# rmazzier/OpenSetGaitRecognition_PCAA

Measured on AMD Instinct MI355X. Metric: gait sequences/sec (train step), higher is better.
Workload: dtype bf16; 1 GPU; PCAA V4 train step (enc+dec+disc fwd/bwd, WGAN-GP, Chamfer, 2x Adam), B=64/GPU T=30 N=128 C=4 K=8, BASELINE config[1]; global_batch=64, precision=bf16, parallelism=dp1, sync_bn=False, finite_loss=True, hip_graph=False, decoder_update=fused wgrad+adam

## Files before the change

include/pcaa_hip.h:

```cpp
#ifndef PCAA_HIP_H
#define PCAA_HIP_H

#include <stddef.h>

#ifdef __cplusplus
extern "C" {
#endif

#define PCAA_ABI_VERSION 27

#define PCAA_OK 0
#define PCAA_ERR_INVALID_ARG 1
#define PCAA_ERR_LAUNCH 2

#define PCAA_F32 0
#define PCAA_BF16 1
#define PCAA_SPLIT_F16 2

#define PCAA_LAYOUT_KC 0
#define PCAA_LAYOUT_RC 1

#define PCAA_ACT_NONE 0
#define PCAA_ACT_ELU 1

const char* pcaa_last_error(void);
int pcaa_abi_version(void);

#define PCAA_GEMM_KERNEL_F32_TILE128 0
#define PCAA_GEMM_KERNEL_BF16_SMALL 1
#define PCAA_GEMM_KERNEL_BF16_STAGED 2
#define PCAA_GEMM_KERNEL_V2_KC 3
#define PCAA_GEMM_KERNEL_V2_RC 4
int pcaa_gemm(int math,
              const void* A, int a_dtype, int a_layout, long lda,
              const void* B, int b_dtype, int b_layout, long ldb,
              void* C, int c_dtype, long ldc,
              int M, int N, int K,
              const float* bias, double* colstats, int nrep,
              int split_k, int accumulate, void* stream);

int pcaa_gemm_num_splits(int math, int K, int split_k);
int pcaa_gemm_route(int math,
                    const void* A, int a_dtype, int a_layout, long lda,
                    const void* B, int b_dtype, int b_layout, long ldb,
                    const void* C, int c_dtype, long ldc,
                    int M, int N, int K,
                    const float* bias, const double* colstats, int nrep,
                    int split_k, int accumulate, long slab_stride);
int pcaa_gemm_split3_route(const void* A, const void* B, int layout, long lda, long ldb, const void* C, long ldc, int M,
                           int N, int K, const double* colstats, int nrep, int split_k, long c_split_stride, float out_scale);
int pcaa_gemm_last_kernel(void);
int pcaa_gemm_group_rc_f32(int n, const void* const* A, const void* const* B, void* const* C, const int* M,
                           const int* N, const int* K, const int* split_k, void* stream);
int pcaa_gemm_group_rc_f32_slabs(int n, const void* const* A, const void* const* B, void* const* slabs, const int* M,
                                 const int* N, const int* K, const int* split_k, void* stream);
int pcaa_gemm_v2_enable(int on);
int pcaa_gemm_slabs(int math,
                    const void* A, int a_dtype, int a_layout, long lda,
                    const void* B, int b_dtype, int b_layout, long ldb,
                    float* slabs, long slab_stride, int M, int N, int K, int split_k, void* stream);
int pcaa_gemm_affine_elu(const void* A, long lda, const void* W, long ldw, void* out, long ldo,
                         const float* scale, const float* shift, int M, int N, int K, int pool_rows,
                         void* stream);
int pcaa_gemm_dgrad_bn_supported(int M, int N, int K);
int pcaa_gemm_dgrad_bn(const void* dy, long lddy, const void* Wt, long ldw, const void* y, void* dz, long ld,
                       const float* scale, const float* shift, const float* mean, const float* rstd,
                       double* stats, int nrep, int M, int N, int K,
                       const float* x, int xc, const float* W1, void* stream);
int pcaa_bn_bwd_dy_split(const float* dz, const float* y, void* dy_img, const float* coef, long rows, int ch,
                         float img_scale, void* stream);
int pcaa_gemm_dgrad_bn_split3(const void* dy_img, long lddy, const void* Wt_img, long ldw, const float* y, float* dz,
                              long ld, const float* scale, const float* shift, const float* mean, const float* rstd,
                              double* stats, int nrep, int M, int N, int K, float out_scale, void* stream);
int pcaa_timing_events_create(void** start, void** stop);
int pcaa_timing_events_destroy(void* start, void* stop);
int pcaa_time_next_gemm(void* start, void* stop);
int pcaa_timing_pending(void);
int pcaa_timing_elapsed_ms(void* start, void* stop, float* ms);
int pcaa_splitk_reduce(const float* slabs, int nsplit, long slab_stride, long n, float* out,
                       int accumulate, void* stream);
int pcaa_splitk_reduce_stats(const float* slabs, int nsplit, long slab_stride, float* out,
                             double* stats, int nrep, long rows, int ch, void* stream);

int pcaa_pointnet_in_fwd(const float* x, int C, const float* W, const float* bias, void* y, int y_dtype,
                         long P, int cout, double* stats, int nrep, void* stream);
int pcaa_pointnet_in_wgrad(const void* dy, int dy_dtype, const float* x, int C, float* dW, long P,
                           int cout, void* stream);
int pcaa_pointnet_in_apply(const float* x, int C, const float* W, const float* scale, const float* shift,
                           void* a, int a_dtype, long P, int cout, void* stream);
int pcaa_pointnet_in_bwd_stats(const void* da, int dtype, const float* x, int C, const float* W,
                               const float* scale, const float* shift, const float* mean, const float* rstd,
                               double* stats, int nrep, long P, int cout, void* stream);
int pcaa_pointnet_in_bwd_onepass(const void* da, int dtype, const float* x, int C, const float* W,
                                 const float* scale, const float* shift, const float* mean, const float* rstd,
                                 double* stats, int nrep, float* G, long P, int cout, const double* pivot_mom,
                                 double pivot_inv_count, void* stream);
int pcaa_pointnet_in_bwd_onepass_rows(const void* da, int dtype, const float* x, int C, const float* W,
                                      const float* scale, const float* shift, const float* mean, const float* rstd,
                                      double* stats, int nrep, float* G, long P, int cout, const double* pivot_mom,
                                      double pivot_inv_count, void* stream);
int pcaa_pointnet_in_bwd_g_rows(long P);
int pcaa_points_moments_size(void);
int pcaa_points_moments(const float* x, int C, long P, double* mom, void* stream);
int pcaa_pointnet_in_bwd_combine(const float* G, int nrep, const float* W, const double* mom, const float* coef,
                                 float* dW, int cout, int C, long P, const double* pivot_mom, double pivot_inv_count,
                                 void* stream);
int pcaa_pointnet_in_moment_stats(const double* mom, const float* W, int C, int cout, void* stream);
int pcaa_pointnet_in_bwd_wgrad(const void* da, int dtype, const float* x, int C, const float* W,
                               const float* scale, const float* shift, const float* coef, float* dW,
                               long P, int cout, int dz_is_pre ,
                               void* stream);

int pcaa_cast_bf16(const float* src, void* dst, void* dst_t, int R, int C, void* stream);

int pcaa_bn_finalize(const double* stats, int nrep, long count, const float* lin_bias,
                     const float* gamma, const float* beta,
                     float* running_mean, float* running_var, long long* num_batches_tracked,
                     float momentum, float eps,
                     float* scale, float* shift, float* mean, float* rstd, int ch, void* stream);
int pcaa_bn_eval_coeffs(const float* gamma, const float* beta, const float* running_mean,
                        const float* running_var, const float* lin_bias, float eps, float* scale,
                        float* shift, int ch, void* stream);
int pcaa_bn_act_fwd(const void* y, void* a, int dtype, const float* scale, const float* shift,
                    long rows, int ch, void* stream);
int pcaa_bn_act_meanpool_fwd(const void* y, int dtype, const float* scale, const float* shift,
                             const float* mean, const float* rstd, float* pooled, float* e1, float* e2,
                             long groups, int group_rows, int ch, void* stream);
int pcaa_bn_pool_bwd_stats(const float* dpool, const float* e1, const float* e2, float pool_scale,
                           double* stats, int nrep, long groups, int ch, void* stream);
int pcaa_bn_act_bwd_dz(const void* da, const float* dpool, int group_rows, float pool_scale,
                       const void* y, void* dz, int dtype,
                       const float* scale, const float* shift, const float* mean, const float* rstd,
                       double* stats, int nrep, long rows, int ch, void* stream);
int pcaa_bn_bwd_finalize(const double* stats, int nrep, long count, const float* gamma,
                         const float* mean, const float* rstd,
                         float* coef, float* dgamma, float* dbeta, int ch, void* stream);
int pcaa_bn_bwd_dy(const void* dz, const void* y, void* dy, int dtype, const float* coef,
                   long rows, int ch, void* stream);
int pcaa_bn_eval_moments(const float* running_mean, const float* running_var, const float* lin_bias,
                         float eps, float* mean, float* rstd, int ch, void* stream);
int pcaa_bn_eval_act_bwd(const void* da, const float* dpool, int group_rows, float pool_scale,
                         const void* y, void* dy, int dtype,
                         const float* scale, const float* shift, const float* mean, const float* rstd,
                         double* stats, int nrep, long rows, int ch, void* stream);
int pcaa_bn_eval_bwd_finalize(const double* stats, int nrep, const float* scale,
                              float* dgamma, float* dbeta, float* dbias, int ch, void* stream);
int pcaa_bn_tail_arm_fwd(const double* stats, int nrep, long count, const float* lin_bias,
                         const float* gamma, const float* beta,
                         float* running_mean, float* running_var, long long* num_batches_tracked,
                         float momentum, float eps,
                         float* scale, float* shift, float* mean, float* rstd, int ch, unsigned* counter);
int pcaa_bn_tail_arm_bwd(const double* stats, int nrep, long count, const float* gamma,
                         const float* mean, const float* rstd,
                         float* coef, float* dgamma, float* dbeta, int ch, unsigned* counter);
int pcaa_bn_tail_pending(void);
int pcaa_bn_tail_disarm(void);
int pcaa_bn_bwd_dy_fused(const void* da, const float* dpool, int group_rows, float pool_scale,
                         const void* y, void* dy, int dtype, const float* scale, const float* shift,
                         const float* coef, long rows, int ch, void* stream);

int pcaa_bias_act(float* y, const float* bias, int act, long rows, int cols, void* stream);
int pcaa_elu_bwd_from_out(const float* da, const float* a, float* dz, long n, void* stream);
int pcaa_colsum(const float* x, float* out, long rows, int cols, void* stream);
int pcaa_sum(const float* x, long n, float scale, float* out, void* stream);
int pcaa_rowsum(const float* x, float* out, long rows, int cols, float scale, void* stream);
int pcaa_scale_by_device_scalar(const float* x, const float* s, float* out, long n, void* stream);
int pcaa_scale_rows(const float* x, const float* s, float* out, long rows, int cols, void* stream);
int pcaa_prior_sample(const float* z0, const float* means, const long long* gt, int B, int K, int D,
                      float* z, float* onehot, void* stream);
int pcaa_pack_points(const float* src, long sb, long sc, long st, long sn,
                     float* dst, int B, int C, int T, int N, void* stream);

int pcaa_gather_rows(const void* src, long n_src_rows, long row_bytes, const long long* idx, void* dst,
                     long n_rows, int* err_flag, void* stream);

int pcaa_dtc_im2col(const float* a, float* col, int B, int T, int Cin, int dilation, void* stream);
int pcaa_dtc_col2im(const float* dcol, float* da, int B, int T, int Cin, int dilation, void* stream);

int pcaa_chamfer_fwd_bwd(const float* preds, long p_sb, long p_sc, long p_st, long p_sn,
                         const float* gts, long g_sb, long g_sc, long g_st, long g_sn,
                         int B, int T, int N, int C, float* frame_loss,
                         float* dpreds, long d_sb, long d_sc, long d_st, long d_sn,
                         float grad_scale, const float* grad_per_b, void* stream);
int pcaa_cross_entropy(const float* logits, const long long* target, int B, int K,
                       float* loss, float* dlogits, float grad_scale, long long* preds,
                       int* err_flag, void* stream);

int pcaa_disc_forward(const float* x, const float* label, int B, int K,
                      const float* W1, const float* b1, const float* W2, const float* b2,
                      const float* W3, const float* b3, float* out, void* stream);
int pcaa_disc_backward(const float* x, const float* label, int B, int K,
                       const float* W1, const float* b1, const float* W2, const float* b2,
                       const float* W3, const float* b3, const float* gout,
                       float* dx, float* dlabel,
                       float* dW1, float* db1, float* dW2, float* db2, float* dW3, float* db3,
                       float* workspace, size_t workspace_bytes, void* stream);
int pcaa_disc_backward_backward(const float* x, const float* label, int B, int K,
                                const float* W1, const float* b1, const float* W2, const float* b2,
                                const float* W3, const float* b3, const float* gout, const float* gbar,
                                float* dx2, float* dlabel2, float* dgout,
                                float* dW1, float* db1, float* dW2, float* db2, float* dW3, float* db3,
                                float* workspace, size_t workspace_bytes, void* stream);
size_t pcaa_disc_workspace_bytes(int B, int K);
int pcaa_disc_wgan_gp(const float* z, const float* fv, const float* label, const float* alphas,
                      int B, int K,
                      const float* W1, const float* b1, const float* W2, const float* b2,
                      const float* W3, const float* b3, float gp_weight, float* losses,
                      float* dW1, float* db1, float* dW2, float* db2, float* dW3, float* db3,
                      float* dz, float* workspace, size_t workspace_bytes, void* stream);

int pcaa_joint_likelihood(const float* x, const float* means, int B, int K, int D, double* lik,
                          void* stream);
int pcaa_kvote(const double* lik, const long long* preds, double threshold, int k, int n_labels,
               int n_classes, int n_windows, long long* out, void* stream);

int pcaa_skinny_supported(int M, int N, int K);
int pcaa_skinny_splits(int kind, int M, int N, int K);
int pcaa_skinny_linear_fwd(const float* x, long ldx, const float* W, long ldw, const float* bias, int act,
                           float* y, float* ws, long ws_floats, int M, int N, int K, int nsplit,
                           void* stream);
int pcaa_skinny_linear_dgrad(const float* dz, long lddz, const float* W, long ldw, float* dx,
// ... 173 lines not shown
```

opensetgaitrecognition_pcaa_amd/csrc/elementwise.hip:

```cpp
#include <stdarg.h>

#include "common.h"
#include "bn_tail.h"

static thread_local char g_err[512] = "";
void pcaa_set_error(const char* fmt, ...) {
  va_list ap;
  va_start(ap, fmt);
  vsnprintf(g_err, sizeof(g_err), fmt, ap);
  va_end(ap);
}
extern "C" const char* pcaa_last_error(void) { return g_err; }
static thread_local int* g_range_flag = nullptr;
int* pcaa_range_flag_ptr() { return g_range_flag; }
extern "C" int pcaa_set_range_flag(int* dev_flag) { g_range_flag = dev_flag; return PCAA_OK; }
extern "C" int pcaa_abi_version(void) { return PCAA_ABI_VERSION; }

namespace {

constexpr int ROWS_PER_BLOCK = 128;

inline bool ch_ok(int ch) {
  if (ch < 4 || ch > 1024 || (ch & 3)) return false;
  const int q = ch >> 2;
  return (256 % q) == 0;
}

__device__ __forceinline__ void replica_sums(const double* __restrict__ stats, int nrep, int ch, int c, double& s1,
                                             double& s2) {
  int r = 0;
  for (; r + 8 <= nrep; r += 8) {
    double a[8], b[8];
#pragma unroll
    for (int u = 0; u < 8; ++u) {
      a[u] = stats[((long)(r + u) * 2 + 0) * ch + c];
      b[u] = stats[((long)(r + u) * 2 + 1) * ch + c];
    }
#pragma unroll
    for (int u = 0; u < 8; ++u) { s1 += a[u]; s2 += b[u]; }
  }
  for (; r < nrep; ++r) {
    s1 += stats[((long)r * 2 + 0) * ch + c];
    s2 += stats[((long)r * 2 + 1) * ch + c];
  }
}

__global__ void bn_finalize_kernel(const double* __restrict__ stats, int nrep, double inv_count,
                                   double unbias, const float* __restrict__ lin_bias,
                                   const float* __restrict__ gamma, const float* __restrict__ beta,
                                   float* running_mean, float* running_var, long long* nbt,
                                   float momentum, float eps, float* scale, float* shift,
                                   float* mean_out, float* rstd_out, int ch) {
  const int c = blockIdx.x * blockDim.x + threadIdx.x;
  if (c == 0 && nbt) *nbt += 1;
  if (c >= ch) return;
  double s1 = 0.0, s2 = 0.0;
  replica_sums(stats, nrep, ch, c, s1, s2);
  const double m0 = s1 * inv_count;
  double var = s2 * inv_count - m0 * m0;
  if (var < 0.0) var = 0.0;
  const double mean = m0 + (lin_bias ? (double)lin_bias[c] : 0.0);
  const double rstd = 1.0 / sqrt(var + (double)eps);
  const float sc = (float)((double)gamma[c] * rstd);
  scale[c] = sc;
  shift[c] = (float)((double)beta[c] - m0 * (double)gamma[c] * rstd);
  mean_out[c] = (float)m0;
  rstd_out[c] = (float)rstd;
  if (running_mean) {
    running_mean[c] = (1.f - momentum) * running_mean[c] + momentum * (float)mean;
    running_var[c] = (1.f - momentum) * running_var[c] + momentum * (float)(var * unbias);
  }
}

__global__ void bn_eval_coeffs_kernel(const float* gamma, const float* beta, const float* rm,
                                      const float* rv, const float* lin_bias, float eps, float* scale,
                                      float* shift, int ch) {
  const int c = blockIdx.x * blockDim.x + threadIdx.x;
  if (c >= ch) return;
  const float rstd = 1.f / sqrtf(rv[c] + eps);
  const float sc = gamma[c] * rstd;
  scale[c] = sc;
  shift[c] = beta[c] + ((lin_bias ? lin_bias[c] : 0.f) - rm[c]) * sc;
}

template <typename T>
__global__ __launch_bounds__(256) void bn_act_fwd_kernel(const T* __restrict__ y, T* __restrict__ a,
// ... 511 lines not shown
    long r = i / Cin;
    const int t = (int)(r % T);
    const long b = r / T;
    float acc = 0.f;
#pragma unroll
    for (int tap = 0; tap < 3; ++tap) {
      const int tt = t + (2 - tap) * d;
      if (tt < T) acc += dcol[((b * T + tt) * Cin + ci) * 3 + tap];
    }
    da[i] = acc;
  }
}

template <int U, typename TG = float>
__global__ __launch_bounds__(256) void adam_kernel(float* __restrict__ p, const TG* __restrict__ g,
                                                   float* __restrict__ m, float* __restrict__ v, long n,
                                                   float b1, float b2, float eps, float step_size,
                                                   float inv_bc2_sqrt, float grad_scale,
                                                   const float* __restrict__ coef) {
  if (coef) {
    step_size = coef[0];
    inv_bc2_sqrt = coef[1];
  }
  const long nq = n >> 2;
  const long stride = (long)gridDim.x * 256;
  for (long q0 = (long)blockIdx.x * 256 + threadIdx.x; q0 < nq; q0 += stride * U) {
    f32x4 pv[U], gv[U], mv[U], vv[U];
#pragma unroll
    for (int u = 0; u < U; ++u) {
      const long q = q0 + u * stride;
      if (q < nq) { pv[u] = load4(p + q * 4); gv[u] = load4(g + q * 4); mv[u] = load4(m + q * 4); vv[u] = load4(v + q * 4); }
    }
#pragma unroll
    for (int u = 0; u < U; ++u) {
      const long q = q0 + u * stride;
      if (q >= nq) break;
#pragma unroll
      for (int e = 0; e < 4; ++e) {
        float pe = pv[u][e], me = mv[u][e], ve = vv[u][e];
        adam_update(pe, me, ve, gv[u][e] * grad_scale, b1, b2, eps, step_size, inv_bc2_sqrt);
        pv[u][e] = pe; mv[u][e] = me; vv[u][e] = ve;
      }
      store4(p + q * 4, pv[u]);
      store4(m + q * 4, mv[u]);
      store4(v + q * 4, vv[u]);
    }
  }
  if (blockIdx.x == 0 && threadIdx.x < (n & 3)) {
    const long i = (nq << 2) + threadIdx.x;
    float pp = p[i], mm = m[i], vv = v[i];
    adam_update(pp, mm, vv, (float)g[i] * grad_scale, b1, b2, eps, step_size, inv_bc2_sqrt);
    m[i] = mm;
    v[i] = vv;
    p[i] = pp;
  }
}

__global__ void adam_coef_kernel(int* __restrict__ step, float* __restrict__ coef, float lr, float b1, float b2) {
  const int t = *step + 1;
  *step = t;
  const double bc1 = 1.0 - pow((double)b1, (double)t);
  const double bc2 = 1.0 - pow((double)b2, (double)t);
  coef[0] = (float)((double)lr / bc1);
  coef[1] = (float)(1.0 / sqrt(bc2));
}

inline int grid_for(long work_items, int per_block = 256, int cap = 256 * 8) {
  long g = cdiv(work_items, per_block);
  if (g < 1) g = 1;
  if (g > cap) g = cap;
  return (int)g;
}

inline int col_invariant_grid(long nquads, int qpr) {
  int a = qpr, b = 256;
  while (b) { const int t = a % b; a = b; b = t; }
  const int unit = qpr / a;
  long g = cdiv(nquads, 256);
  if (g > 2048) g = 2048;
  g = cdiv(g, unit) * unit;
  return (int)g;
}

}

extern "C" int pcaa_bn_finalize(const double* stats, int nrep, long count, const float* lin_bias,
                                const float* gamma, const float* beta, float* running_mean,
                                float* running_var, long long* num_batches_tracked, float momentum,
                                float eps, float* scale, float* shift, float* mean, float* rstd,
                                int ch, void* stream) {
  PCAA_CHECK_ARG(stats && gamma && beta && scale && shift && mean && rstd, "pcaa_bn_finalize: null pointer");
  PCAA_CHECK_ARG(nrep >= 1 && count >= 1 && ch >= 1, "pcaa_bn_finalize: bad sizes");
  PCAA_CHECK_ARG((running_mean == nullptr) == (running_var == nullptr), "pcaa_bn_finalize: running stats must come together");
  const double unbias = count > 1 ? (double)count / (double)(count - 1) : 1.0;
  hipLaunchKernelGGL(bn_finalize_kernel, dim3((unsigned)cdiv(ch, 256)), dim3(256), 0, as_stream(stream),
                     stats, nrep, 1.0 / (double)count, unbias, lin_bias, gamma, beta, running_mean,
                     running_var, num_batches_tracked, momentum, eps, scale, shift, mean, rstd, ch);
  PCAA_RETURN_LAUNCH_STATUS("pcaa_bn_finalize");
}

extern "C" int pcaa_bn_eval_coeffs(const float* gamma, const float* beta, const float* running_mean,
                                   const float* running_var, const float* lin_bias, float eps, float* scale,
                                   float* shift, int ch, void* stream) {
  PCAA_CHECK_ARG(gamma && beta && running_mean && running_var && scale && shift && ch >= 1, "pcaa_bn_eval_coeffs: bad args");
  hipLaunchKernelGGL(bn_eval_coeffs_kernel, dim3((unsigned)cdiv(ch, 256)), dim3(256), 0, as_stream(stream),
                     gamma, beta, running_mean, running_var, lin_bias, eps, scale, shift, ch);
  PCAA_RETURN_LAUNCH_STATUS("pcaa_bn_eval_coeffs");
}

extern "C" int pcaa_bn_act_fwd(const void* y, void* a, int dtype, const float* scale, const float* shift,
                               long rows, int ch, void* stream) {
  PCAA_CHECK_ARG(y && a && scale && shift, "pcaa_bn_act_fwd: null pointer");
  PCAA_CHECK_ARG(rows >= 1 && ch >= 4 && (ch & 3) == 0, "pcaa_bn_act_fwd: ch must be a multiple of 4");
  const long nq = rows * (ch >> 2);
  PCAA_CHECK_ARG(nq < (1L << 31), "pcaa_bn_act_fwd: tensor too large for 32-bit quad indices");
  const int grid = col_invariant_grid(nq, ch >> 2);
  if (dtype == PCAA_F32)
    hipLaunchKernelGGL(bn_act_fwd_kernel<float>, dim3(grid), dim3(256), 0, as_stream(stream),
                       (const float*)y, (float*)a, scale, shift, (unsigned)nq, (unsigned)(ch >> 2));
  else if (dtype == PCAA_BF16)
    hipLaunchKernelGGL(bn_act_fwd_kernel<bf16_t>, dim3(grid), dim3(256), 0, as_stream(stream),
                       (const bf16_t*)y, (bf16_t*)a, scale, shift, (unsigned)nq, (unsigned)(ch >> 2));
  else { pcaa_set_error("pcaa_bn_act_fwd: bad dtype"); return PCAA_ERR_INVALID_ARG; }
  PCAA_RETURN_LAUNCH_STATUS("pcaa_bn_act_fwd");
}

extern "C" int pcaa_bn_act_fwd_split(const float* y, void* a_img, const float* scale, const float* shift, long rows,
                                     int ch, float img_scale, void* stream) {
  PCAA_CHECK_ARG(y && a_img && scale && shift, "pcaa_bn_act_fwd_split: null pointer");
  PCAA_CHECK_ARG(rows >= 1 && ch >= 4 && (ch & 3) == 0, "pcaa_bn_act_fwd_split: ch must be a multiple of 4");
  const long nq = rows * (ch >> 2);
  PCAA_CHECK_ARG(nq < (1L << 31), "pcaa_bn_act_fwd_split: tensor too large for 32-bit quad indices");
  const int grid = col_invariant_grid(nq, ch >> 2);
  hipLaunchKernelGGL(bn_act_fwd_split_kernel, dim3(grid), dim3(256), 0, as_stream(stream), y, (split_t*)a_img, scale, shift,
                     (unsigned)nq, (unsigned)(ch >> 2), img_scale, pcaa_range_flag_ptr());
  PCAA_RETURN_LAUNCH_STATUS("pcaa_bn_act_fwd_split");
}

extern "C" int pcaa_split_f16(const float* src, void* dst_img, long rows, int ch, int transpose, float img_scale,
                               void* stream) {
  PCAA_CHECK_ARG(src && dst_img && rows >= 1 && ch >= 1, "pcaa_split_f16: bad args");
  long g = cdiv(rows * ch, 256);
  if (g > 4096) g = 4096;
  hipLaunchKernelGGL(split_f16_kernel, dim3((unsigned)g), dim3(256), 0, as_stream(stream), src, (split_t*)dst_img, rows, ch,
                     transpose, img_scale, pcaa_range_flag_ptr());
  PCAA_RETURN_LAUNCH_STATUS("pcaa_split_f16");
}

extern "C" int pcaa_bn_act_meanpool_fwd(const void* y, int dtype, const float* scale, const float* shift,
                                        const float* mean, const float* rstd, float* pooled, float* e1, float* e2,
                                        long groups, int group_rows, int ch, void* stream) {
  PCAA_CHECK_ARG(y && scale && shift && pooled, "pcaa_bn_act_meanpool_fwd: null pointer");
  PCAA_CHECK_ARG(groups >= 1 && group_rows >= 1 && ch_ok(ch), "pcaa_bn_act_meanpool_fwd: ch/4 must divide 256 (ch=%d)", ch);
  const bool train = e1 != nullptr;
  PCAA_CHECK_ARG((e2 != nullptr) == train && (!train || (mean && rstd)),
                 "pcaa_bn_act_meanpool_fwd: e1, e2, mean, rstd come together");
  hipStream_t s = as_stream(stream);
#define LAUNCH_MP(T, TRAIN)                                                                                   \
  hipLaunchKernelGGL((bn_act_meanpool_kernel<T, TRAIN>), dim3((unsigned)groups), dim3(256), 0, s, (const T*)y, \
                     scale, shift, mean, rstd, pooled, e1, e2, group_rows, ch)
  if (dtype == PCAA_BF16 && ch == 1024 && group_rows % 4 == 0 && groups >= 512) {
    const unsigned grid = (unsigned)std::min<long>(groups, 1024);
    if (train)
      hipLaunchKernelGGL(bn_act_meanpool_stream_kernel<true>, dim3(grid), dim3(256), 0, s, (const bf16_t*)y, scale, shift,
                         mean, rstd, pooled, e1, e2, groups, group_rows, ch);
    else
      hipLaunchKernelGGL(bn_act_meanpool_stream_kernel<false>, dim3(grid), dim3(256), 0, s, (const bf16_t*)y, scale, shift,
                         mean, rstd, pooled, e1, e2, groups, group_rows, ch);
  }
  else if (dtype == PCAA_F32) { if (train) LAUNCH_MP(float, true); else LAUNCH_MP(float, false); }
  else if (dtype == PCAA_BF16) { if (train) LAUNCH_MP(bf16_t, true); else LAUNCH_MP(bf16_t, false); }
  else { pcaa_set_error("pcaa_bn_act_meanpool_fwd: bad dtype"); return PCAA_ERR_INVALID_ARG; }
#undef LAUNCH_MP
  PCAA_RETURN_LAUNCH_STATUS("pcaa_bn_act_meanpool_fwd");
}

extern "C" int pcaa_bn_pool_bwd_stats(const float* dpool, const float* e1, const float* e2, float pool_scale,
                                      double* stats, int nrep, long groups, int ch, void* stream) {
  PCAA_CHECK_ARG(dpool && e1 && e2 && stats, "pcaa_bn_pool_bwd_stats: null pointer");
  PCAA_CHECK_ARG(groups >= 1 && ch >= 4 && (ch & 3) == 0 && nrep >= 1, "pcaa_bn_pool_bwd_stats: ch must be a multiple of 4");
  const int gpb = (int)std::max<long>(1, std::min<long>(32, groups / 256));
  hipLaunchKernelGGL(bn_pool_bwd_stats_kernel, dim3((unsigned)cdiv(groups, gpb)), dim3(256), 0, as_stream(stream),
                     dpool, e1, e2, pool_scale, stats, nrep, groups, ch, gpb, pcaa_take_bn_tail(stats));
  PCAA_RETURN_LAUNCH_STATUS("pcaa_bn_pool_bwd_stats");
}

extern "C" int pcaa_bn_act_bwd_dz(const void* da, const float* dpool, int group_rows, float pool_scale,
                                  const void* y, void* dz, int dtype, const float* scale,
                                  const float* shift, const float* mean, const float* rstd,
                                  double* stats, int nrep, long rows, int ch, void* stream) {
  PCAA_CHECK_ARG((da != nullptr) != (dpool != nullptr), "pcaa_bn_act_bwd_dz: exactly one of da / dpool");
  PCAA_CHECK_ARG(y && scale && shift && mean && rstd && stats, "pcaa_bn_act_bwd_dz: null pointer");
  PCAA_CHECK_ARG(rows >= 1 && rows < (1L << 31) && nrep >= 1 && ch_ok(ch),
                 "pcaa_bn_act_bwd_dz: ch/4 must divide 256 (ch=%d), rows < 2^31", ch);
  PCAA_CHECK_ARG(!dpool || group_rows >= 1, "pcaa_bn_act_bwd_dz: bad group_rows");
  const unsigned grid = (unsigned)cdiv(rows, ROWS_PER_BLOCK);
  hipStream_t s = as_stream(stream);
#define LAUNCH_DZ(T, POOL)                                                                       \
// ... 138 lines not shown
  PCAA_CHECK_ARG(rows >= 1 && rows < (1L << 31) && nrep >= 1 && ch_ok(ch),
                 "pcaa_bn_eval_act_bwd: ch/4 must divide 256 (ch=%d), rows < 2^31", ch);
  PCAA_CHECK_ARG(!dpool || group_rows >= 1, "pcaa_bn_eval_act_bwd: bad group_rows");
  PCAA_CHECK_ARG(dy != y, "pcaa_bn_eval_act_bwd: dy may alias da, not y");
  const unsigned grid = (unsigned)cdiv(rows, ROWS_PER_BLOCK);
  hipStream_t s = as_stream(stream);
#define LAUNCH_EV(T, POOL)                                                                         \
  hipLaunchKernelGGL((bn_eval_act_bwd_kernel<T, POOL>), dim3(grid), dim3(256), 0, s, (const T*)da, \
                     dpool, (unsigned)group_rows, pool_scale, (const T*)y, (T*)dy, scale, shift,   \
                     mean, rstd, stats, nrep, rows, ch)
  if (dtype == PCAA_F32) { if (dpool) LAUNCH_EV(float, true); else LAUNCH_EV(float, false); }
  else if (dtype == PCAA_BF16) { if (dpool) LAUNCH_EV(bf16_t, true); else LAUNCH_EV(bf16_t, false); }
  else { pcaa_set_error("pcaa_bn_eval_act_bwd: bad dtype"); return PCAA_ERR_INVALID_ARG; }
#undef LAUNCH_EV
  PCAA_RETURN_LAUNCH_STATUS("pcaa_bn_eval_act_bwd");
}

extern "C" int pcaa_bn_eval_bwd_finalize(const double* stats, int nrep, const float* scale, float* dgamma,
                                         float* dbeta, float* dbias, int ch, void* stream) {
  PCAA_CHECK_ARG(stats && (scale || !dbias), "pcaa_bn_eval_bwd_finalize: null pointer");
  PCAA_CHECK_ARG(nrep >= 1 && ch >= 1, "pcaa_bn_eval_bwd_finalize: bad sizes");
  hipLaunchKernelGGL(bn_eval_bwd_finalize_kernel, dim3((unsigned)cdiv(ch, 256)), dim3(256), 0, as_stream(stream),
                     stats, nrep, scale, dgamma, dbeta, dbias, ch);
  PCAA_RETURN_LAUNCH_STATUS("pcaa_bn_eval_bwd_finalize");
}

namespace {
thread_local BnTail g_tail = {};
}
BnTail pcaa_take_bn_tail(const double* stats) {
  BnTail t = {};
  if (g_tail.kind != 0 && g_tail.stats == stats) {
    t = g_tail;
    g_tail.kind = 0;
  }
  return t;
}
extern "C" int pcaa_bn_tail_arm_fwd(const double* stats, int nrep, long count, const float* lin_bias,
                                    const float* gamma, const float* beta, float* running_mean, float* running_var,
                                    long long* num_batches_tracked, float momentum, float eps, float* scale,
                                    float* shift, float* mean, float* rstd, int ch, unsigned* counter) {
  PCAA_CHECK_ARG(stats && gamma && beta && scale && shift && mean && rstd && counter, "pcaa_bn_tail_arm_fwd: null pointer");
  PCAA_CHECK_ARG(nrep >= 1 && count >= 1 && ch >= 1, "pcaa_bn_tail_arm_fwd: bad sizes");
  PCAA_CHECK_ARG((running_mean == nullptr) == (running_var == nullptr), "pcaa_bn_tail_arm_fwd: running stats must come together");
  BnTail t = {};
  t.kind = 1; t.nrep = nrep; t.ch = ch; t.counter = counter; t.stats = stats;
  t.inv_count = 1.0 / (double)count;
  t.unbias = count > 1 ? (double)count / (double)(count - 1) : 1.0;
  t.lin_bias = lin_bias; t.gamma = gamma; t.beta = beta;
  t.running_mean = running_mean; t.running_var = running_var; t.nbt = num_batches_tracked;
  t.momentum = momentum; t.eps = eps;
  t.scale = scale; t.shift = shift; t.mean = mean; t.rstd = rstd;
  g_tail = t;
  return PCAA_OK;
}
extern "C" int pcaa_bn_tail_arm_bwd(const double* stats, int nrep, long count, const float* gamma, const float* mean,
                                    const float* rstd, float* coef, float* dgamma, float* dbeta, int ch,
                                    unsigned* counter) {
  PCAA_CHECK_ARG(stats && gamma && mean && rstd && coef && counter, "pcaa_bn_tail_arm_bwd: null pointer");
  PCAA_CHECK_ARG(nrep >= 1 && count >= 1 && ch >= 1, "pcaa_bn_tail_arm_bwd: bad sizes");
  BnTail t = {};
  t.kind = 2; t.nrep = nrep; t.ch = ch; t.counter = counter; t.stats = stats;
  t.inv_count = 1.0 / (double)count;
  t.gamma = gamma; t.mean = const_cast<float*>(mean); t.rstd = const_cast<float*>(rstd);
  t.coef = coef; t.dgamma = dgamma; t.dbeta = dbeta;
  g_tail = t;
  return PCAA_OK;
}
void pcaa_rearm_bn_tail(const BnTail& t) {
  if (t.kind != 0) g_tail = t;
}
extern "C" int pcaa_bn_tail_pending(void) { return g_tail.kind != 0 ? 1 : 0; }
extern "C" int pcaa_bn_tail_disarm(void) {
  g_tail.kind = 0;
  return PCAA_OK;
}

extern "C" int pcaa_bn_bwd_dy(const void* dz, const void* y, void* dy, int dtype, const float* coef,
                              long rows, int ch, void* stream) {
  PCAA_CHECK_ARG(dz && y && dy && coef, "pcaa_bn_bwd_dy: null pointer");
  PCAA_CHECK_ARG(rows >= 1 && ch >= 4 && (ch & 3) == 0, "pcaa_bn_bwd_dy: ch must be a multiple of 4");
  const long nq = rows * (ch >> 2);
  PCAA_CHECK_ARG(nq < (1L << 31), "pcaa_bn_bwd_dy: tensor too large for 32-bit quad indices");
  const int grid = col_invariant_grid(nq, ch >> 2);
  if (dtype == PCAA_F32)
    hipLaunchKernelGGL(bn_bwd_dy_kernel<float>, dim3(grid), dim3(256), 0, as_stream(stream), (const float*)dz,
                       (const float*)y, (float*)dy, coef, (unsigned)nq, (unsigned)(ch >> 2), (unsigned)ch);
  else if (dtype == PCAA_BF16)
    hipLaunchKernelGGL(bn_bwd_dy_kernel<bf16_t>, dim3(grid), dim3(256), 0, as_stream(stream), (const bf16_t*)dz,
                       (const bf16_t*)y, (bf16_t*)dy, coef, (unsigned)nq, (unsigned)(ch >> 2), (unsigned)ch);
  else { pcaa_set_error("pcaa_bn_bwd_dy: bad dtype"); return PCAA_ERR_INVALID_ARG; }
  PCAA_RETURN_LAUNCH_STATUS("pcaa_bn_bwd_dy");
}

extern "C" int pcaa_bn_bwd_dy_split(const float* dz, const float* y, void* dy_img, const float* coef, long rows, int ch,
                                    float img_scale, void* stream) {
  PCAA_CHECK_ARG(dz && y && dy_img && coef, "pcaa_bn_bwd_dy_split: null pointer");
  PCAA_CHECK_ARG(rows >= 1 && ch >= 4 && (ch & 3) == 0, "pcaa_bn_bwd_dy_split: ch must be a multiple of 4");
  PCAA_CHECK_ARG((const void*)dz != dy_img && (const void*)y != dy_img, "pcaa_bn_bwd_dy_split: the image cannot alias an input");
  const long nq = rows * (ch >> 2);
  PCAA_CHECK_ARG(nq < (1L << 31), "pcaa_bn_bwd_dy_split: tensor too large for 32-bit quad indices");
  const int grid = col_invariant_grid(nq, ch >> 2);
  hipLaunchKernelGGL(bn_bwd_dy_split_kernel, dim3(grid), dim3(256), 0, as_stream(stream), dz, y, (split_t*)dy_img, coef,
                     (unsigned)nq, (unsigned)(ch >> 2), (unsigned)ch, img_scale, pcaa_range_flag_ptr());
  PCAA_RETURN_LAUNCH_STATUS("pcaa_bn_bwd_dy_split");
}

extern "C" int pcaa_bias_act(float* y, const float* bias, int act, long rows, int cols, void* stream) {
  PCAA_CHECK_ARG(y && rows >= 1 && cols >= 1, "pcaa_bias_act: bad args");
  PCAA_CHECK_ARG(act == PCAA_ACT_NONE || act == PCAA_ACT_ELU, "pcaa_bias_act: bad activation");
  const long n = rows * cols;
  hipLaunchKernelGGL(bias_act_kernel, dim3(grid_for(n)), dim3(256), 0, as_stream(stream), y, bias, act, n, cols);
  PCAA_RETURN_LAUNCH_STATUS("pcaa_bias_act");
}

extern "C" int pcaa_elu_bwd_from_out(const float* da, const float* a, float* dz, long n, void* stream) {
  PCAA_CHECK_ARG(da && a && dz && n >= 1, "pcaa_elu_bwd_from_out: bad args");
  hipLaunchKernelGGL(elu_bwd_from_out_kernel, dim3(grid_for(n)), dim3(256), 0, as_stream(stream), da, a, dz, n);
  PCAA_RETURN_LAUNCH_STATUS("pcaa_elu_bwd_from_out");
}

extern "C" int pcaa_colsum(const float* x, float* out, long rows, int cols, void* stream) {
  PCAA_CHECK_ARG(x && out && rows >= 1 && cols >= 1, "pcaa_colsum: bad args");
  hipLaunchKernelGGL(colsum_kernel, dim3((unsigned)cdiv(cols, 64)), dim3(256), 0, as_stream(stream), x, out, rows, cols);
  PCAA_RETURN_LAUNCH_STATUS("pcaa_colsum");
}

extern "C" int pcaa_sum(const float* x, long n, float scale, float* out, void* stream) {
  PCAA_CHECK_ARG(x && out && n >= 1, "pcaa_sum: bad args");
  hipLaunchKernelGGL(sum_kernel, dim3(1), dim3(1024), 0, as_stream(stream), x, n, scale, out);
  PCAA_RETURN_LAUNCH_STATUS("pcaa_sum");
}

extern "C" int pcaa_rowsum(const float* x, float* out, long rows, int cols, float scale, void* stream) {
  PCAA_CHECK_ARG(x && out && rows >= 1 && cols >= 1, "pcaa_rowsum: bad args");
  hipLaunchKernelGGL(rowsum_kernel, dim3((unsigned)rows), dim3(64), 0, as_stream(stream), x, out, cols, scale);
  PCAA_RETURN_LAUNCH_STATUS("pcaa_rowsum");
}

extern "C" int pcaa_scale_by_device_scalar(const float* x, const float* s, float* out, long n, void* stream) {
  PCAA_CHECK_ARG(x && s && out && n >= 1, "pcaa_scale_by_device_scalar: bad args");
  hipLaunchKernelGGL(scale_dev_kernel, dim3(grid_for(n)), dim3(256), 0, as_stream(stream), x, s, out, n);
  PCAA_RETURN_LAUNCH_STATUS("pcaa_scale_by_device_scalar");
}

extern "C" int pcaa_scale_rows(const float* x, const float* s, float* out, long rows, int cols, void* stream) {
  PCAA_CHECK_ARG(x && s && out && rows >= 1 && cols >= 1, "pcaa_scale_rows: bad args");
  const long n = rows * cols;
  hipLaunchKernelGGL(scale_rows_kernel, dim3(grid_for(n)), dim3(256), 0, as_stream(stream), x, s, out, n, cols);
  PCAA_RETURN_LAUNCH_STATUS("pcaa_scale_rows");
}

extern "C" int pcaa_prior_sample(const float* z0, const float* means, const long long* gt, int B, int K, int D,
                                 float* z, float* onehot, void* stream) {
  PCAA_CHECK_ARG(z0 && means && gt && z && onehot && B >= 1 && K >= 1 && D >= 1, "pcaa_prior_sample: bad args");
  const int n = B * (D > K ? D : K);
  hipLaunchKernelGGL(prior_sample_kernel, dim3((unsigned)cdiv(n, 256)), dim3(256), 0, as_stream(stream), z0, means, gt, B, K, D, z, onehot);
  PCAA_RETURN_LAUNCH_STATUS("pcaa_prior_sample");
}

extern "C" int pcaa_pack_points(const float* src, long sb, long sc, long st, long sn, float* dst,
                                int B, int C, int T, int N, void* stream) {
  PCAA_CHECK_ARG(src && dst && B >= 1 && C >= 1 && T >= 1 && N >= 1, "pcaa_pack_points: bad args");
  const long n = (long)B * C * T * N;
  hipLaunchKernelGGL(pack_points_kernel, dim3(grid_for(n)), dim3(256), 0, as_stream(stream), src, sb, sc, st, sn, dst, B, C, T, N);
  PCAA_RETURN_LAUNCH_STATUS("pcaa_pack_points");
// ... 177 lines not shown
```

Before: 12310 sequences/s.

## Add persistent ring-buffered streaming kernel for bf16 BN act-fwd and bwd-dy

Adds a persistent-grid streaming kernel that keeps per-column coefficients in registers and software-pipelines 16-byte bf16 loads through a small register ring (depth 2-4). The bf16 BN backward dy path and the wide-channel (ch>=1024) activation forward path use it, with nontemporal loads and stores on the backward path. The grid is sized per CU count. The aim is higher memory bandwidth utilisation on these bandwidth-bound elementwise passes, at the cost of extra code paths gated by alignment and channel-divisibility checks and an environment toggle.

After: 12440 sequences/s (median of 6 runs). 1.01x the previous value.

```diff
diff --git a/include/pcaa_hip.h b/include/pcaa_hip.h
--- a/include/pcaa_hip.h
+++ b/include/pcaa_hip.h
@@ -7,7 +7,7 @@
 extern "C" {
 #endif
 
-#define PCAA_ABI_VERSION 27
+#define PCAA_ABI_VERSION 28
 
 #define PCAA_OK 0
 #define PCAA_ERR_INVALID_ARG 1
@@ -137,6 +137,16 @@
                          float* coef, float* dgamma, float* dbeta, int ch, void* stream);
 int pcaa_bn_bwd_dy(const void* dz, const void* y, void* dy, int dtype, const float* coef,
                    long rows, int ch, void* stream);
+#define PCAA_EW_ACT_FWD 0
+#define PCAA_EW_BWD_DY 1
+#define PCAA_EW_BWD_DY_FUSED 2
+#define PCAA_EW_MEANPOOL 3
+#define PCAA_EW_IN_BWD 4
+#define PCAA_EW_IN_APPLY 5
+const char* pcaa_ew_route(int pass, int dtype, long rows, int ch, int aligned);
+int pcaa_ew_wgs_per_cu(int pass);
+int pcaa_ew_ring_depth(int pass);
+int pcaa_ew_stream_set(int on);
 int pcaa_bn_eval_moments(const float* running_mean, const float* running_var, const float* lin_bias,
                          float eps, float* mean, float* rstd, int ch, void* stream);
 int pcaa_bn_eval_act_bwd(const void* da, const float* dpool, int group_rows, float pool_scale,
diff --git a/opensetgaitrecognition_pcaa_amd/csrc/elementwise.hip b/opensetgaitrecognition_pcaa_amd/csrc/elementwise.hip
--- a/opensetgaitrecognition_pcaa_amd/csrc/elementwise.hip
+++ b/opensetgaitrecognition_pcaa_amd/csrc/elementwise.hip
@@ -1,7 +1,10 @@
 #include <stdarg.h>
+
+#include <stdlib.h>
 
 #include "common.h"
 #include "bn_tail.h"
+#include "ew_stream.h"
 
 static thread_local char g_err[512] = "";
 void pcaa_set_error(const char* fmt, ...) {
@@ -679,6 +682,49 @@
   return (int)g;
 }
 
+int g_ew_stream = -1;
+inline bool ew_stream_on() {
+  if (g_ew_stream < 0) {
+    const char* e = getenv("PCAA_EW_STREAM");
+    g_ew_stream = (e && e[0] == '0' && e[1] == 0) ? 0 : 1;
+  }
+  return g_ew_stream != 0;
+}
+inline bool ew_route_stream(int pass, int dtype, long rows, int ch, bool aligned16) {
+  if (!ew_stream_on() || dtype != PCAA_BF16 || rows < 1 || !aligned16 || !ew::ch_ok(ch)) return false;
+  if (pass == PCAA_EW_ACT_FWD) return ch >= 1024;
+  return pass == PCAA_EW_BWD_DY;
+}
+inline bool aligned16(const void* a, const void* b, const void* c) {
+  return (((uintptr_t)a | (uintptr_t)b | (uintptr_t)c) & 15) == 0;
+}
+
+}
+
+int ew::cu_count() {
+  static int n = 0;
+  if (n <= 0) {
+    int dev = 0;
+    if (hipGetDevice(&dev) != hipSuccess || hipDeviceGetAttribute(&n, hipDeviceAttributeMultiprocessorCount, dev) != hipSuccess ||
+        n <= 0)
+      n = 256;
+  }
+  return n;
+}
+
+extern "C" const char* pcaa_ew_route(int pass, int dtype, long rows, int ch, int aligned) {
+  return ew_route_stream(pass, dtype, rows, ch, aligned != 0) ? "stream" : "classic";
+}
+extern "C" int pcaa_ew_wgs_per_cu(int pass) {
+  return pass == PCAA_EW_ACT_FWD ? ew::ActFwdPolicy::K : pass == PCAA_EW_BWD_DY ? ew::BwdDyPolicy::K : 0;
+}
+extern "C" int pcaa_ew_ring_depth(int pass) {
+  return pass == PCAA_EW_ACT_FWD ? ew::ActFwdPolicy::R : pass == PCAA_EW_BWD_DY ? ew::BwdDyPolicy::R : 0;
+}
+extern "C" int pcaa_ew_stream_set(int on) {
+  const int was = ew_stream_on() ? 1 : 0;
+  g_ew_stream = on ? 1 : 0;
+  return was;
 }
 
 extern "C" int pcaa_bn_finalize(const double* stats, int nrep, long count, const float* lin_bias,
@@ -711,6 +757,11 @@
   PCAA_CHECK_ARG(rows >= 1 && ch >= 4 && (ch & 3) == 0, "pcaa_bn_act_fwd: ch must be a multiple of 4");
   const long nq = rows * (ch >> 2);
   PCAA_CHECK_ARG(nq < (1L << 31), "pcaa_bn_act_fwd: tensor too large for 32-bit quad indices");
+  if (ew_route_stream(PCAA_EW_ACT_FWD, dtype, rows, ch, aligned16(y, a, nullptr))) {
+    ew::launch<1, ew::ActFwdPolicy>((const bf16_t*)y, nullptr, (bf16_t*)a, ew::ActFwd{scale, shift}, rows, ch,
+                                    as_stream(stream));
+    PCAA_RETURN_LAUNCH_STATUS("pcaa_bn_act_fwd");
+  }
   const int grid = col_invariant_grid(nq, ch >> 2);
   if (dtype == PCAA_F32)
     hipLaunchKernelGGL(bn_act_fwd_kernel<float>, dim3(grid), dim3(256), 0, as_stream(stream),
@@ -1015,6 +1066,11 @@
   PCAA_CHECK_ARG(rows >= 1 && ch >= 4 && (ch & 3) == 0, "pcaa_bn_bwd_dy: ch must be a multiple of 4");
   const long nq = rows * (ch >> 2);
   PCAA_CHECK_ARG(nq < (1L << 31), "pcaa_bn_bwd_dy: tensor too large for 32-bit quad indices");
+  if (ew_route_stream(PCAA_EW_BWD_DY, dtype, rows, ch, aligned16(dz, y, dy))) {
+    ew::launch<2, ew::BwdDyPolicy>((const bf16_t*)y, (const bf16_t*)dz, (bf16_t*)dy, ew::BwdDy{coef}, rows, ch,
+                                   as_stream(stream));
+    PCAA_RETURN_LAUNCH_STATUS("pcaa_bn_bwd_dy");
+  }
   const int grid = col_invariant_grid(nq, ch >> 2);
   if (dtype == PCAA_F32)
     hipLaunchKernelGGL(bn_bwd_dy_kernel<float>, dim3(grid), dim3(256), 0, as_stream(stream), (const float*)dz,
diff --git a/opensetgaitrecognition_pcaa_amd/csrc/ew_stream.h b/opensetgaitrecognition_pcaa_amd/csrc/ew_stream.h
--- /dev/null
+++ b/opensetgaitrecognition_pcaa_amd/csrc/ew_stream.h
@@ -0,0 +1,117 @@
+#pragma once
+#include "common.h"
+
+namespace ew {
+
+typedef unsigned int u32x2 __attribute__((ext_vector_type(2)));
+typedef unsigned int u32x4 __attribute__((ext_vector_type(4)));
+
+constexpr int OCT = 8;
+
+inline bool ch_ok(int ch) { return ch >= OCT && (ch % OCT) == 0 && ch / OCT <= 256 && (256 % (ch / OCT)) == 0; }
+inline int rows_per_trip(int ch) { return 256 / (ch / OCT); }
+
+__device__ __forceinline__ f32x4 unpack(unsigned lo, unsigned hi) {
+  return f32x4{__uint_as_float(lo << 16), __uint_as_float(lo & 0xffff0000u), __uint_as_float(hi << 16),
+               __uint_as_float(hi & 0xffff0000u)};
+}
+__device__ __forceinline__ u32x2 pack(f32x4 v) {
+  bf16x4 b;
+  b.x = (bf16_t)v.x; b.y = (bf16_t)v.y; b.z = (bf16_t)v.z; b.w = (bf16_t)v.w;
+  return __builtin_bit_cast(u32x2, b);
+}
+template <bool NT>
+__device__ __forceinline__ u32x4 load16(const bf16_t* p) {
+  if (NT) return __builtin_nontemporal_load(reinterpret_cast<const u32x4*>(p));
+  return *reinterpret_cast<const u32x4*>(p);
+}
+template <bool NT>
+__device__ __forceinline__ void store16(bf16_t* p, u32x4 v) {
+  if (NT) __builtin_nontemporal_store(v, reinterpret_cast<u32x4*>(p));
+  else *reinterpret_cast<u32x4*>(p) = v;
+}
+
+template <int NIN, int R, bool NTL, bool NTS, typename F>
+__global__ __launch_bounds__(256) void stream_kernel(const bf16_t* __restrict__ in0, const bf16_t* in1, bf16_t* out, F f,
+                                                     unsigned rows, unsigned ch) {
+  const unsigned L = ch / OCT, rpt = 256u / L;
+  const unsigned c = (threadIdx.x % L) * OCT, rl = threadIdx.x / L;
+  const unsigned G = gridDim.x, full = rows / rpt;
+  typename F::Coef k;
+  f.init(k, c, ch);
+  u32x4 b0[R], b1[R];
+  auto issue = [&](int s, unsigned t) {
+    const unsigned row = min(t * rpt + rl, rows - 1);
+    const size_t o = (size_t)row * ch + c;
+    b0[s] = load16<NTL>(in0 + o);
+    if (NIN == 2) b1[s] = load16<NTL>(in1 + o);
+  };
+  auto consume = [&](int s, unsigned t, bool refill, bool all_rows) {
+    const unsigned row = t * rpt + rl;
+    const u32x4 w0 = b0[s], w1 = NIN == 2 ? b1[s] : b0[s];
+    const u32x2 lo = pack(f.quad(k, 0, unpack(w0.x, w0.y), unpack(w1.x, w1.y)));
+    const u32x2 hi = pack(f.quad(k, 1, unpack(w0.z, w0.w), unpack(w1.z, w1.w)));
+    if (refill) issue(s, t + R * G);
+    if (all_rows || row < rows) store16<NTS>(out + (size_t)row * ch + c, u32x4{lo.x, lo.y, hi.x, hi.y});
+  };
+  unsigned t = blockIdx.x;
+#pragma unroll
+  for (int s = 0; s < R; ++s) issue(s, t + s * G);
+  for (; t + (R - 1) * G < full; t += R * G) {
+#pragma unroll
+    for (int s = 0; s < R; ++s) consume(s, t + s * G, true, true);
+  }
+#pragma unroll
+  for (int s = 0; s < R; ++s) consume(s, t + s * G, false, false);
+}
+
+struct ActFwd {
+  const float *scale, *shift;
+  struct Coef { f32x4 sc[2], sh[2]; };
+  __device__ __forceinline__ void init(Coef& k, unsigned c, unsigned) const {
+    k.sc[0] = load4(scale + c); k.sc[1] = load4(scale + c + 4);
+    k.sh[0] = load4(shift + c); k.sh[1] = load4(shift + c + 4);
+  }
+  __device__ __forceinline__ f32x4 quad(const Coef& k, int h, f32x4 v, f32x4) const {
+    f32x4 o;
+    o.x = elu_t<bf16_t>(__builtin_fmaf(v.x, k.sc[h].x, k.sh[h].x));
+    o.y = elu_t<bf16_t>(__builtin_fmaf(v.y, k.sc[h].y, k.sh[h].y));
+    o.z = elu_t<bf16_t>(__builtin_fmaf(v.z, k.sc[h].z, k.sh[h].z));
+    o.w = elu_t<bf16_t>(__builtin_fmaf(v.w, k.sc[h].w, k.sh[h].w));
+    return o;
+  }
+};
+
+struct BwdDy {
+  const float* coef;
+  struct Coef { f32x4 k0[2], k1[2], k2[2]; };
+  __device__ __forceinline__ void init(Coef& k, unsigned c, unsigned ch) const {
+#pragma unroll
+    for (int h = 0; h < 2; ++h) {
+      k.k0[h] = load4(coef + c + 4 * h);
+      k.k1[h] = load4(coef + ch + c + 4 * h);
+      k.k2[h] = load4(coef + 2 * ch + c + 4 * h);
+    }
+  }
+  __device__ __forceinline__ f32x4 quad(const Coef& k, int h, f32x4 yv, f32x4 d) const {
+#pragma clang fp contract(off)
+    const f32x4 t = k.k1[h] * yv;
+    return __builtin_elementwise_fma(k.k0[h], d, t) + k.k2[h];
+  }
+};
+
+struct ActFwdPolicy { static constexpr int K = 2, R = 2; static constexpr bool NTL = false, NTS = false; };
+struct BwdDyPolicy { static constexpr int K = 1, R = 4; static constexpr bool NTL = true, NTS = true; };
+
+int cu_count();
+
+template <int NIN, typename P, typename F>
+inline void launch(const bf16_t* in0, const bf16_t* in1, bf16_t* out, const F& f, long rows, int ch, hipStream_t stream) {
+  const long trips = cdiv(rows, rows_per_trip(ch));
+  long grid = (long)P::K * cu_count();
+  if (grid > trips) grid = trips;
+  hipLaunchKernelGGL((stream_kernel<NIN, P::R, P::NTL, P::NTS, F>), dim3((unsigned)grid), dim3(256), 0, stream, in0, in1,
+                     out, f, (unsigned)rows, (unsigned)ch);
+}
+
+}
```
